# igd-geo/schwarzwald

Hardware: AMD Instinct MI355X
Metric: Mpoints/s end-to-end tile (Morton+sort+sample) (higher is better)
Workload: dtype u64 keys / f64 positions

## Files before the change

### schwarzwald_amd/csrc/swz_level.h

```cpp
#pragma once
#include "swz_device.h"
#include "swz_internal.h"

namespace swz {

enum : uint8_t { MODE_TAKE_ALL = 0, MODE_SAMPLE = 1 };

enum {
  CTR_NUM_NODES = 0,
  CTR_SAMPLE_NODES = 1,
  CTR_SAMPLE_POINTS = 2,
  CTR_ERROR = 3,
  CTR_REMAINING = 4,
  CTR_NUM_CELLS = 5,
  CTR_DONE_CELLS = 6,
  CTR_Q0 = 8,
  CTR_DBG_TIME = 20,
  CTR_DBG_TMAX = 21,
  CTR_DBG_HIST = 22,
  CTR_COUNT = 40
};

struct ActiveSet {
  const uint64_t* akey = nullptr;
// ... 59 lines not shown

LevelPlan make_plan(int level, int sampler, uint64_t max_points, float spacing_at_root, uint32_t max_depth,
                    const double bmin[3], const double bmax[3], bool force_sample, bool tiler_rules);
int alloc_level_buffers(swz_ctx* c, uint32_t m, LevelBuffers* lb);
int required_depth_host(int sampler, int node_level, double root_extent_x, float root_max_spacing);
int level_step(swz_ctx* c, const LevelPlan& plan, const ActiveSet& as, const SortedPoints& sp, const LevelBuffers& lb,
               int8_t* level_out, uint64_t* okey, uint32_t* oidx, LevelResult* res);
int fast_start_level(swz_ctx* c, const uint64_t* d_keys_sorted, uint32_t n, uint32_t concurrency, int* start_level);
int fast_prefix_counts(swz_ctx* c, const uint64_t* d_keys_sorted, uint32_t n, uint32_t* counts_host);
int fast_start_level_from_counts(const uint64_t* counts, uint32_t concurrency);

int min_distance_level(swz_ctx* c, const LevelPlan& plan, const ActiveSet& as, const SortedPoints& sp,
                       const LevelBuffers& lb, uint32_t num_nodes, uint32_t sample_nodes,
                       uint32_t sample_points, uint32_t* rounds_out);

int min_distance_property_level(swz_ctx* c, const LevelPlan& plan, const ActiveSet& as, const SortedPoints& sp,
                                const LevelBuffers& lb, uint32_t num_nodes, uint32_t sample_nodes,
                                uint32_t sample_points, uint32_t* phases_out);

struct MdPeerView {
  const uint4* rec = nullptr;
  const uint64_t* qpos = nullptr;
  const uint8_t* state = nullptr;
  const float4* ovf = nullptr;
  const uint32_t* gridmap = nullptr;
  const uint32_t* round_word = nullptr;
  const uint32_t* perm = nullptr;
  const double* xyz = nullptr;
  const uint32_t* aidx = nullptr;
  uint32_t ncells = 0, rg = 0, cell_shift = 0;
  uint32_t npoints = 0;
  int status = 0;
  int entered = 0;
};
struct MdShardRoot {
  int shard = 0, shards = 1;
  MdPeerView* views = nullptr;
  void (*barrier)(void*) = nullptr;
  void* barrier_arg = nullptr;
};

struct KeyMetric {
  bool ok = false;
  double T = 0.0;
  float f_lo = 0.f;
  float f_hi = 0.f;
};
KeyMetric key_metric(const swz_ctx* c, const LevelPlan& plan, const SortedPoints& sp);
int key_point_ids(swz_ctx* c, const ActiveSet& as, const SortedPoints& sp, const uint32_t** ids);
bool min_distance_level_uses_keys(const swz_ctx* c, const LevelPlan& plan, const SortedPoints& sp);
bool level_decides_on_keys(const swz_ctx* c, const LevelPlan& plan, const SortedPoints& sp);
int min_distance_keys_level(swz_ctx* c, const LevelPlan& plan, const ActiveSet& as, const SortedPoints& sp,
                            const LevelBuffers& lb, uint32_t num_nodes, uint32_t sample_nodes, uint32_t sample_points,
                            const uint32_t* snode_of, int cl, double typical_pop, uint32_t* rounds_out, bool* used,
                            const MdShardRoot* shard_root = nullptr);

int min_distance_rounds_level(swz_ctx* c, const LevelPlan& plan, const ActiveSet& as, const SortedPoints& sp, const LevelBuffers& lb,
                              uint32_t num_nodes, uint32_t sample_nodes, uint32_t sample_points, const uint32_t* snode_of, uint32_t* rounds_out,
                              bool* used);

int min_distance_sparse_level(swz_ctx* c, const LevelPlan& plan, const ActiveSet& as, const SortedPoints& sp,
                              const LevelBuffers& lb, const uint32_t* snode_of, bool all_sampled, uint32_t num_nodes,
                              uint32_t sample_nodes, uint32_t sample_points, const uint32_t occupied[12], uint32_t* rounds_out,
                              bool* used);

int min_distance_block_level(swz_ctx* c, const LevelPlan& plan, const ActiveSet& as, const SortedPoints& sp, const LevelBuffers& lb,
                             const uint32_t* snode_of, bool all_sampled, uint32_t num_nodes, uint32_t sample_nodes,
                             uint32_t sample_points, const uint32_t occupied[12], const KeyMetric& km, bool* done);

}
```

### schwarzwald_amd/csrc/swz_mdkeys.hip

```cpp
#include <algorithm>
#include <chrono>
#include <cmath>
#include <cstdio>
#include <cstdlib>
#include <cstring>
#include <string>
#include <vector>

#include "swz_level.h"
#include "swz_scan.h"

namespace swz {

constexpr uint32_t QNONE = 0xFFFFFFFFu;
constexpr unsigned long long QEMPTY = ~0ull;
constexpr uint32_t MQ_WOKEN = 0x80000000u;
constexpr int MQ_LIST_CAP = 128;
constexpr int MQ_FRESH_CAP = 32;
#ifndef MQ_MINW4
#define MQ_MINW4 4
#endif
#ifndef MQ_MINW1
#define MQ_MINW1 6
#endif
// ... 32 lines not shown
  return k;
}

__global__ __launch_bounds__(256) void mq_point_ids_kernel(const uint32_t* __restrict__ aidx, const uint32_t* __restrict__ perm, uint32_t m,
                                                           uint32_t ghosts, uint32_t* __restrict__ ids) {
  const uint32_t i = blockIdx.x * 256 + threadIdx.x;
  if (i >= m) return;
  const uint32_t s = aidx ? aidx[i] : i;
  ids[i] = s < ghosts ? perm[s] : ghosts + perm[s];
}
int key_point_ids(swz_ctx* c, const ActiveSet& as, const SortedPoints& sp, const uint32_t** ids) {
  if (!as.aidx && !sp.ghosts) {
    *ids = sp.perm;
    return SWZ_OK;
  }
  uint32_t* d = nullptr;
  SWZ_TRY(c->get("md_qids", (size_t)as.m, &d));
  hipLaunchKernelGGL(mq_point_ids_kernel, dim3(div_up(as.m, 256)), dim3(256), 0, c->stream, as.aidx, sp.perm, as.m, sp.ghosts, d);
  SWZ_LAUNCH_CHECK(c);
  *ids = d;
  return SWZ_OK;
}

constexpr uint32_t MQ_PEER_SHIFT = 28;
constexpr uint32_t MQ_ID_MASK = (1u << MQ_PEER_SHIFT) - 1u;
struct MqPeers {
  const uint4* rec[8];
  const uint64_t* qpos[8];
  const uint8_t* state[8];
  const float4* ovf[8];
  const uint32_t* gridmap[8];
  const uint32_t* round_word[8];
  const uint32_t* perm[8];
  const double* xyz[8];
  const uint32_t* aidx[8];
  uint32_t shard, shards;
};

struct MqArgs {
  const uint64_t* akey;
  const uint32_t* aidx;
  uint32_t m;
  const uint32_t* nid;
  const uint8_t* nmode;
  const uint32_t* nstart;
  const double* xyz;
  const uint32_t* perm;
  const double* gxyz;
  uint32_t ng;
  uint8_t* taken;
  uint32_t* counters;
  uint64_t* qpos;
  uint8_t* state;
  uint2* cinfo;
  uint32_t* crel;
  uint32_t* csnode;
  uint32_t* gridmap;
  uint32_t* qnbr;
  uint4* rec;
  float4* ovf;
  unsigned long long* slot;
  uint4* qst;
  uint32_t* queue[2];
  uint32_t* qctr;
  uint32_t* qtotal;
  uint32_t* qhead;
  uint32_t nseg, nseg_shift, segcap;
  const uint32_t* snode_of;
  uint32_t cell_shift;
  uint64_t cells_per_node;
  uint32_t cell_bits;
  uint32_t cell_levels;
  uint32_t rg, rg2_shift;
  float f_lo, f_hi;
  double sq_spacing;
  uint32_t patient;
  float lazy_frac;
  uint32_t all_sampled;
  uint32_t group, groups;
  uint32_t no_dead_test;
  uint32_t stats;
  uint32_t chain;
  uint32_t dense_min;
  uint8_t* dirty;
  uint32_t* bulk_round;
  const uint32_t* dlist;
  uint32_t* round_word;
  MqPeers peers;
};

__device__ __forceinline__ uint32_t uni(uint32_t v) { return (uint32_t)__builtin_amdgcn_readfirstlane((int)v); }
__device__ __forceinline__ uint32_t qb_u32(uint32_t v, int src) { return (uint32_t)__builtin_amdgcn_readlane((int)v, src); }
__device__ __forceinline__ float qb_f32(float v, int src) {
  return __int_as_float(__builtin_amdgcn_readlane(__float_as_int(v), src));
}
__device__ __forceinline__ unsigned long long qb_u64(unsigned long long v, int src) {
  const uint32_t lo = qb_u32((uint32_t)v, src), hi = qb_u32((uint32_t)(v >> 32), src);
  return ((unsigned long long)hi << 32) | lo;
}
template <typename Op>
__device__ __forceinline__ uint32_t mq_wave_scan(uint32_t v, Op op, uint32_t identity) {
  v = op(v, (uint32_t)__builtin_amdgcn_update_dpp((int)identity, (int)v, 0x111, 0xF, 0xF, false));
  v = op(v, (uint32_t)__builtin_amdgcn_update_dpp((int)identity, (int)v, 0x112, 0xF, 0xF, false));
  v = op(v, (uint32_t)__builtin_amdgcn_update_dpp((int)identity, (int)v, 0x114, 0xF, 0xF, false));
  v = op(v, (uint32_t)__builtin_amdgcn_update_dpp((int)identity, (int)v, 0x118, 0xF, 0xF, false));
  v = op(v, (uint32_t)__builtin_amdgcn_update_dpp((int)identity, (int)v, 0x142, 0xA, 0xF, false));
// ... 55 lines not shown
__device__ __forceinline__ uint32_t mq_ld_sys(const uint32_t* p) { return __hip_atomic_load(p, __ATOMIC_RELAXED, __HIP_MEMORY_SCOPE_SYSTEM); }

__device__ __forceinline__ bool mq_exact_near_peer(const MqArgs& a, uint32_t i, uint32_t j, uint32_t tag) {
  const double* p = sorted_point_xyz(a.xyz, a.perm, a.gxyz, a.ng, a.aidx ? a.aidx[i] : i);
  const double* q = tag ? a.peers.xyz[tag - 1u] + (size_t)a.peers.perm[tag - 1u][a.peers.aidx[tag - 1u] ? a.peers.aidx[tag - 1u][j] : j] * 3
                        : sorted_point_xyz(a.xyz, a.perm, a.gxyz, a.ng, a.aidx ? a.aidx[j] : j);
  return sq_dist(p[0], p[1], p[2], q[0], q[1], q[2]) < a.sq_spacing;
}

struct MqLds {
  uint4* stage;
  float4* list;
  float4* fresh;
  uint8_t* tag;
  uint32_t* trust;
  uint32_t* sid;
};
constexpr uint32_t MQ_CHAIN = 8;
__host__ __device__ constexpr uint32_t mq_staged(bool peers) { return peers ? 27u : 20u; }
static inline size_t mq_lds_bytes(uint32_t rg, bool peers) {
  return (size_t)(mq_staged(peers) * 2u * rg + MQ_LIST_CAP + MQ_FRESH_CAP) * 16u + MQ_LIST_CAP + MQ_CHAIN * 4u + 128u;
}

__device__ __forceinline__ bool mq_is_head(const MqArgs& a, uint32_t i) {
  if (!a.all_sampled && a.nmode[a.nid[i]] != MODE_SAMPLE) return false;
  return i == 0 || ((a.akey[i] >> a.cell_shift) != (a.akey[i - 1] >> a.cell_shift));
}

__global__ __launch_bounds__(256) void mq_pack_kernel(const uint64_t* __restrict__ akey, uint32_t m, uint64_t* __restrict__ qpos,
                                                      uint8_t* __restrict__ state) {
  const uint32_t i = blockIdx.x * 256 + threadIdx.x;
  if (i >= m) return;
  qpos[i] = mq_pack(akey[i]);
  state[i] = QS_OPEN;
}

struct MqHeadF {
  MqArgs a;
  __device__ uint32_t operator()(uint32_t i) const { return mq_is_head(a, i) ? 1u : 0u; }
};
struct MqCellBuildG {
  MqArgs a;
  __device__ void operator()(uint32_t i, uint32_t c, uint32_t head) const {
    const uint64_t key = a.akey[i];
    a.qpos[i] = mq_pack(key);
    a.state[i] = QS_OPEN;
    if (!head) return;
    a.cinfo[c].x = i;
    a.crel[c] = (uint32_t)((key >> a.cell_shift) & (a.cells_per_node - 1ull));
    a.csnode[c] = a.all_sampled ? a.nid[i] : a.snode_of[a.nid[i]];
  }
};

__global__ __launch_bounds__(256) void mq_cell_end_kernel(MqArgs a, uint32_t ncells) {
  const uint32_t c = blockIdx.x * 256 + threadIdx.x;
  if (c >= ncells) return;
  const uint32_t s = a.cinfo[c].x;
  const uint32_t node_end = a.nstart[a.nid[s] + 1];
  const uint32_t next = (c + 1 < ncells) ? a.cinfo[c + 1].x : a.m;
  const uint32_t e = next < node_end ? next : node_end;
  a.cinfo[c].y = e;
  a.gridmap[(uint64_t)a.csnode[c] * a.cells_per_node + a.crel[c]] = c;
  uint4* r = a.rec + ((size_t)c << a.rg2_shift);
  r[0] = make_uint4(s, 0u, 0u, e);
  r[a.rg] = make_uint4(s, 0u, 1u, e);
  a.qst[c] = make_uint4(QNONE, 0u, 0u, 0u);
}

__device__ __forceinline__ void mq_wave_push(bool want, uint32_t value, uint32_t* qout, uint32_t* cout) {
  const uint64_t m = __ballot(want);
  if (!m) return;
  const int leader = __ffsll((unsigned long long)m) - 1;
  uint32_t base = 0;
  if ((int)lane_id() == leader) base = atomicAdd(cout, (uint32_t)__popcll(m));
  base = __shfl(base, leader, WAVE);
  if (want) qout[base + (uint32_t)__popcll(m & lanemask_lt())] = value;
}

struct MqStart {
  uint32_t* queue[8];
  uint32_t* qctr[8];
  uint32_t groups;
  uint32_t lazy;
};

__global__ __launch_bounds__(256) void mq_nbr_build_kernel(MqArgs a, uint32_t ncells, MqStart st) {
  for (uint64_t cbase = (uint64_t)blockIdx.x * 8u; cbase < ncells; cbase += (uint64_t)gridDim.x * 8u) {
    const uint32_t c = (uint32_t)cbase + threadIdx.x / 32u;
    const uint32_t k = threadIdx.x & 31u;
    const bool in = c < ncells;
    uint32_t nb = QNONE;
    if (in && k == 13u) {
      nb = c;
    } else if (in && k < 27u) {
      const uint32_t rel = a.crel[c];
      const uint32_t all = (uint32_t)(a.cells_per_node - 1ull);
      const uint32_t mz = all & 0x09249249u, my = mz << 1, mx = mz << 2;
      const uint32_t v[3] = {rel & mx, rel & my, rel & mz};
      const uint32_t mk[3] = {mx, my, mz};
      const uint32_t d[3] = {k / 9u, (k / 3u) % 3u, k % 3u};
      bool inside = true;
      uint32_t nrel = 0;
#pragma unroll
      for (int ax = 0; ax < 3; ++ax) {
        uint32_t w = v[ax];
        if (d[ax] == 0u) {
          inside &= w != 0u;
          w = (w - 1u) & mk[ax];
        } else if (d[ax] == 2u) {
          inside &= w != mk[ax];
          w = ((w | ~mk[ax]) + 1u) & mk[ax];
        }
        nrel |= w;
      }
      if (inside) {
        if (a.peers.shards > 1u) {
          const uint32_t owner = (nrel >> (3u * (a.cell_levels - 1u))) * a.peers.shards / 8u;
          if (owner == a.peers.shard) {
            nb = a.gridmap[nrel];
          } else if (owner < a.peers.shard && a.peers.gridmap[owner]) {
            const uint32_t id = a.peers.gridmap[owner][nrel];
            if (id != QNONE) nb = ((owner + 1u) << MQ_PEER_SHIFT) | id;
          }
        } else {
          nb = a.gridmap[(uint64_t)a.csnode[c] * a.cells_per_node + nrel];
        }
      }
    }
    if (in) a.qnbr[(size_t)c * 32 + k] = nb;
    uint32_t best = 0;
    if (st.lazy && in && k < 27u && nb != QNONE && (a.peers.shards <= 1u || (nb >> MQ_PEER_SHIFT) == 0u) && nb < c) best = nb + 1u;
    if (st.lazy) {
#pragma unroll
      for (int off = 16; off >= 1; off >>= 1) best = max(best, (uint32_t)__shfl_xor((int)best, off, 32));
      if (in && best && nb + 1u == best) {
        const uint2 o = a.cinfo[best - 1u];
        const uint32_t bq = o.x + (uint32_t)((float)(o.y - 1u - o.x) * a.lazy_frac);
        a.slot[(size_t)(best - 1u) * 32 + (26u - k)] = (unsigned long long)bq;
        a.qst[c] = make_uint4(a.cinfo[c].x, k, bq, 0u);
      }
    }
    const bool push = in && k == 13u && best == 0u;
    const uint32_t seg = (uint32_t)(cbase >> 3) & (a.nseg - 1u);
    if (st.groups == 1u) {
      mq_wave_push(push, c | MQ_WOKEN, st.queue[0] + (size_t)seg * a.segcap, st.qctr[0] + (size_t)seg * 32u);
    } else {
      const uint32_t g = push ? a.csnode[c] % st.groups : 0u;
      for (uint32_t gg = 0; gg < st.groups; ++gg)
        mq_wave_push(push && g == gg, c | MQ_WOKEN, st.queue[gg] + (size_t)seg * a.segcap, st.qctr[gg] + (size_t)seg * 32u);
    }
  }
}

template <int SU>
__device__ __forceinline__ uint32_t mq_scan(const MqArgs& a, const uint64_t* __restrict__ qpos, const uint8_t* __restrict__ state,
                                            const MqLds& lds, uint32_t live_wn, uint32_t qs, uint32_t qe, float cx, float cy, float cz) {
  const uint32_t l = lane_id();
  for (uint32_t q0 = qs; q0 < qe; q0 += (uint32_t)SU * WAVE) {
    uint64_t v[SU];
    uint8_t s[SU];
#pragma unroll
    for (int u = 0; u < SU; ++u) {
      const uint32_t q = q0 + (uint32_t)u * WAVE + l;
      const bool inb = q < qe;
      v[u] = inb ? qpos[q] : 0ull;
      s[u] = inb ? state[q] : (uint8_t)QS_DEAD;
    }
#pragma unroll
    for (int u = 0; u < SU; ++u) {
      float x, y, z;
      mq_unpack(v[u], x, y, z);
      bool hit = s[u] != QS_DEAD && mq_d2(x, y, z, cx, cy, cz) < a.f_hi;
      uint64_t hb = __ballot(hit);
      if (hb && live_wn) {
        if (hit) {
          for (uint32_t i = 0; i < live_wn; ++i) {
            const float4 e = lds.list[i];
            if (mq_d2(x, y, z, e.x, e.y, e.z) < a.f_lo) {
              hit = false;
              break;
            }
          }
        }
        hb = __ballot(hit);
      }
      if (hb) return q0 + (uint32_t)u * WAVE + (uint32_t)__ffsll((unsigned long long)hb) - 1u;
    }
  }
  return QNONE;
}

__device__ __forceinline__ uint32_t mq_first_open(const uint8_t* __restrict__ state, uint32_t q0, uint32_t qe) {
  const uint32_t l = lane_id();
  while (q0 < qe) {
    const uint32_t base = q0 & ~15u;
    const uint32_t at = base + l * 16u;
    uint4 sb = make_uint4(0x02020202u, 0x02020202u, 0x02020202u, 0x02020202u);
    if (at < qe) sb = *reinterpret_cast<const uint4*>(state + at);
    const uint32_t w[4] = {sb.x, sb.y, sb.z, sb.w};
    uint32_t first = 16u;
// ... 644 lines not shown
    const uint32_t nb = a.qnbr[(size_t)c * 32 + tid];
    if (nb != QNONE && nb <= c) {
      const uint4* r = a.rec + ((size_t)nb << rg2s);
      const uint4 a0 = r[0], a1 = r[rg];
      const uint32_t pick = a1.z > a0.z ? 1u : 0u;
      const uint4 hd = pick ? a1 : a0;
      if (hd.z >= since && hd.y) {
        const uint32_t at = atomicAdd(&cnt, hd.y);
        for (uint32_t j = 0; j < hd.y && at + j < MQ_DENSE_LIST; ++j) {
          uint4 en;
          if (j < cap) en = r[pick * rg + 1u + j];
          else en = *reinterpret_cast<const uint4*>(a.ovf + (hd.w - 1u - (j - cap)));
          lst[at + j] = make_float4(__uint_as_float(en.x), __uint_as_float(en.y), __uint_as_float(en.z), 0.f);
        }
      }
    }
  }
  __syncthreads();
  const uint32_t n = cnt < MQ_DENSE_LIST ? cnt : MQ_DENSE_LIST;
  if (!n) return;
  for (uint32_t p = P + tid; p < e; p += 256u) {
    if (a.state[p] != QS_OPEN) continue;
    float x, y, z;
    mq_unpack(a.qpos[p], x, y, z);
    bool dead = false;
    for (uint32_t i = 0; i < n && !dead; ++i) dead = mq_d2(x, y, z, lst[i].x, lst[i].y, lst[i].z) < a.f_lo;
    if (dead) a.state[p] = QS_DEAD;
  }
}

__global__ void mq_round_word_kernel(uint32_t* word, uint32_t value) {
  __hip_atomic_store(word, value, __ATOMIC_RELAXED, __HIP_MEMORY_SCOPE_SYSTEM);
}

__global__ __launch_bounds__(256) void mq_verify_kernel(MqArgs a, uint32_t ncells, uint32_t* __restrict__ open_cells) {
  const uint32_t c = blockIdx.x * 256 + threadIdx.x;
  bool open = false;
  if (c < ncells) {
    const uint4* r = a.rec + ((size_t)c << a.rg2_shift);
    const uint4 h0 = r[0], h1 = r[a.rg];
    const uint4 h = h1.z > h0.z ? h1 : h0;
    open = h.x < h.w;
  }
  const uint64_t bm = __ballot(open);
  if (bm && lane_id() == 0) atomicAdd(open_cells, (uint32_t)__popcll(bm));
}

bool min_distance_level_uses_keys(const swz_ctx* c, const LevelPlan& plan, const SortedPoints& sp) {
  return key_metric(c, plan, sp).ok;
}

int min_distance_keys_level(swz_ctx* c, const LevelPlan& plan, const ActiveSet& as, const SortedPoints& sp, const LevelBuffers& lb,
                            uint32_t nnodes, uint32_t sample_nodes, uint32_t sample_points, const uint32_t* snode_of, int cl,
                            double typical_pop, uint32_t* rounds_out, bool* used, const MdShardRoot* shard_root) {
  *used = false;
  const KeyMetric km = key_metric(c, plan, sp);
  if (!km.ok) return SWZ_OK;
  const bool sharded = shard_root != nullptr && shard_root->shards > 1;
  const std::string sfx = sharded ? "_sr" : "";
  const uint32_t m = as.m;
  MqArgs a{};
  a.akey = as.akey;
  a.aidx = as.aidx;
  a.m = m;
  a.nid = lb.nid;
  a.nmode = lb.nmode;
  a.nstart = lb.nstart;
  a.xyz = sp.xyz;
  a.perm = sp.perm;
  a.gxyz = sp.ghost_xyz;
  a.ng = sp.ghosts;
  a.taken = lb.taken;
  a.counters = lb.counters;
  a.snode_of = snode_of;
  a.cells_per_node = 1ull << (3 * cl);
  a.cell_levels = (uint32_t)cl;
  a.peers.shards = sharded ? (uint32_t)shard_root->shards : 1u;
  a.peers.shard = sharded ? (uint32_t)shard_root->shard : 0u;
  a.cell_shift = (plan.node_shift == 63u ? 63u : plan.node_shift) - 3u * (uint32_t)cl;
  a.cell_bits = a.cell_shift / 3u;
  a.f_lo = km.f_lo;
  a.f_hi = km.f_hi;
  a.sq_spacing = plan.sq_spacing;
  a.all_sampled = sample_nodes == nnodes ? 1u : 0u;
  a.no_dead_test = c->opt_on("SWZ_MD_NO_DEAD_TEST", false) ? 1u : 0u;
  a.stats = c->opt("SWZ_MD_STATS") ? 1u : 0u;
  a.chain = std::min<uint32_t>(MQ_CHAIN, (uint32_t)std::max(1L, c->opt_int("SWZ_MD_CHAIN", 2)));
  if (a.cell_bits > 21u) return SWZ_OK;

  ProfScope ps(c, "sample_min_distance", (uint64_t)sample_points * 33ull, 1);
  uint32_t* d_cell_sums = nullptr;
  SWZ_TRY(fused_scan_sums(c, MqHeadF{a}, m, lb.counters + CTR_NUM_CELLS, "mqc", &d_cell_sums));
  uint32_t ncells = 0;
  SWZ_HIP(c, hipMemcpyAsync(&ncells, lb.counters + CTR_NUM_CELLS, 4, hipMemcpyDeviceToHost, c->stream));
  SWZ_HIP(c, hipStreamSynchronize(c->stream));
  *used = true;
  if (ncells == 0) return SWZ_OK;
  if (ncells >= 0x7FFFFFFFu) {
    *used = false;
    return SWZ_OK;
  }
  const double r_cell = std::ldexp(1.0, (int)a.cell_bits) / km.T;
  a.rg = (0.75 * r_cell * r_cell * r_cell <= 12.0) ? 4u : 8u;
  a.rg = c->opt_int("SWZ_MD_KEYS_RG", a.rg) >= 8 ? 8u : 4u;
  a.rg2_shift = a.rg == 4u ? 3u : 4u;

  SWZ_TRY(c->get(("md_qpos" + sfx).c_str(), (size_t)m, &a.qpos));
  SWZ_TRY(c->get(("md_qstate" + sfx).c_str(), (size_t)m, &a.state));
  SWZ_TRY(c->get(("md_qovf" + sfx).c_str(), (size_t)m, &a.ovf));
  SWZ_TRY(c->get(("md_qcinfo" + sfx).c_str(), (size_t)ncells, &a.cinfo));
  uint32_t* cellbuf = nullptr;
  SWZ_TRY(c->get(("md_qcells" + sfx).c_str(), (size_t)ncells * 2, &cellbuf));
  a.crel = cellbuf;
  a.csnode = cellbuf + ncells;
  SWZ_TRY(c->get(("md_qnbr" + sfx).c_str(), (size_t)ncells * 32, &a.qnbr));
  SWZ_TRY(c->get(("md_qrec" + sfx).c_str(), (size_t)ncells * 2 * a.rg, &a.rec));
  SWZ_TRY(c->get(("md_qslot" + sfx).c_str(), (size_t)ncells * 32, &a.slot));
  SWZ_TRY(c->get(("md_qst" + sfx).c_str(), (size_t)ncells, &a.qst));
  const uint64_t grid_entries = (uint64_t)sample_nodes * a.cells_per_node;
  SWZ_TRY(c->get(("md_gridmap" + sfx).c_str(), (size_t)grid_entries, &a.gridmap));
  SWZ_HIP(c, memset_large(a.gridmap, 0xFF, (size_t)grid_entries * 4, c->stream));
  SWZ_HIP(c, memset_large(a.slot, 0xFF, (size_t)ncells * 32 * sizeof(unsigned long long), c->stream));

  SWZ_TRY(fused_scan_apply(c, MqHeadF{a}, MqCellBuildG{a}, m, d_cell_sums));
  const uint32_t cb = div_up(ncells, 256);
  hipLaunchKernelGGL(mq_cell_end_kernel, dim3(cb), dim3(256), 0, c->stream, a, ncells);
  SWZ_LAUNCH_CHECK(c);
  struct WordGuard {
    swz_ctx* c;
    uint32_t* word = nullptr;
    bool done = false;
    ~WordGuard() {
      if (word && !done) {
        hipLaunchKernelGGL(mq_round_word_kernel, dim3(1), dim3(1), 0, c->stream, word, MQ_ROUND_FAILED);
        (void)hipStreamSynchronize(c->stream);
      }
    }
  } word_guard{c};
  if (sharded) {
    MdPeerView& mine = shard_root->views[shard_root->shard];
    int my_status = SWZ_OK;
    if (cl < 1 || ncells >= (1u << MQ_PEER_SHIFT) || sample_nodes != 1) my_status = SWZ_ERR_INTERNAL;
    const uint32_t* aidx_sr = nullptr;
    if (as.aidx) {
      uint32_t* cp = nullptr;
      SWZ_TRY(c->get("md_qaidx_sr", (size_t)m, &cp));
      SWZ_HIP(c, hipMemcpyAsync(cp, as.aidx, (size_t)m * 4, hipMemcpyDeviceToDevice, c->stream));
      aidx_sr = cp;
    }
    SWZ_TRY(c->get("md_qround_sr", (size_t)32, &a.round_word));
    hipLaunchKernelGGL(mq_round_word_kernel, dim3(1), dim3(1), 0, c->stream, a.round_word, MQ_FIRST_ROUND);
    SWZ_LAUNCH_CHECK(c);
    SWZ_HIP(c, hipStreamSynchronize(c->stream));
    mine.rec = a.rec;
    mine.qpos = a.qpos;
    mine.state = a.state;
    mine.ovf = a.ovf;
    mine.gridmap = a.gridmap;
    mine.round_word = a.round_word;
    mine.perm = a.perm;
    mine.xyz = a.xyz;
    mine.aidx = aidx_sr;
    mine.ncells = ncells;
    mine.npoints = m;
    mine.rg = a.rg;
    mine.cell_shift = a.cell_shift;
    mine.status = my_status;
    mine.entered = 1;
    word_guard.word = a.round_word;
    shard_root->barrier(shard_root->barrier_arg);
    for (int p = 0; p < shard_root->shards; ++p) {
      const MdPeerView& v = shard_root->views[p];
      if (v.status != SWZ_OK || (v.ncells && (v.rg != a.rg || v.cell_shift != a.cell_shift)))
        return c->fail(SWZ_ERR_INTERNAL, "MIN_DISTANCE root of a sharded batch: shard " + std::to_string(p) +
                                           " cannot take part in the joint sweep (cell levels, cell count or record size differ)");
      if (p < shard_root->shard && v.ncells) {
        a.peers.rec[p] = v.rec;
        a.peers.qpos[p] = v.qpos;
        a.peers.state[p] = v.state;
        a.peers.ovf[p] = v.ovf;
        a.peers.gridmap[p] = v.gridmap;
        a.peers.round_word[p] = v.round_word;
        a.peers.perm[p] = v.perm;
        a.peers.xyz[p] = v.xyz;
        a.peers.aidx[p] = v.aidx;
      }
    }
  }
  const bool many_small = ncells >= (4u << 20) && (double)sample_points / (double)ncells <= 128.0;
  a.patient = (uint32_t)c->opt_int("SWZ_MD_PATIENT", many_small ? 1 : 0);
  const bool lazy = c->opt_on("SWZ_MD_LAZY", true);
  a.lazy_frac = (float)c->opt_num("SWZ_MD_LAZY_FRAC", many_small ? 0.5 : 0.0);
  const bool big_cells = c->opt_on("SWZ_MD_BIG", typical_pop > 256.0);
  uint32_t groups = 1;
  if (sample_nodes >= 2 && !big_cells) groups = 2;
  groups = (uint32_t)std::max(1L, std::min(8L, c->opt_int("SWZ_MD_GROUPS", groups)));
  groups = std::min(groups, sample_nodes);
  if (sharded) groups = 1;
  uint32_t ndense = 0;
  a.dense_min = 0;
  a.dirty = nullptr;
  if (big_cells && groups == 1 && !sharded) {
    const uint32_t dense_min = (uint32_t)std::max(0L, c->opt_int("SWZ_MD_DENSE_MIN", 4096));
    if (dense_min && m >= dense_min) {
      uint32_t* dl = nullptr;
      uint32_t* dcount = nullptr;
      SWZ_TRY(c->get("md_qdense", (size_t)(m / dense_min + 1u), &dl));
      SWZ_TRY(c->get("md_qdense_count", (size_t)4, &dcount));
      SWZ_HIP(c, hipMemsetAsync(dcount, 0, 4, c->stream));
      a.dense_min = dense_min;
      hipLaunchKernelGGL(mq_dense_list_kernel, dim3(cb), dim3(256), 0, c->stream, a, ncells, dl, dcount);
      SWZ_LAUNCH_CHECK(c);
      SWZ_HIP(c, hipMemcpyAsync(&ndense, dcount, 4, hipMemcpyDeviceToHost, c->stream));
      SWZ_HIP(c, hipStreamSynchronize(c->stream));
      if (ndense) {
        SWZ_TRY(c->get("md_qdirty", (size_t)ncells, &a.dirty));
        SWZ_TRY(c->get("md_qbulk", (size_t)ncells, &a.bulk_round));
        SWZ_HIP(c, hipMemsetAsync(a.dirty, 0, (size_t)ncells, c->stream));
        SWZ_HIP(c, hipMemsetAsync(a.bulk_round, 0, (size_t)ncells * 4, c->stream));
        a.dlist = dl;
      } else {
        a.dense_min = 0;
      }
    }
  }
  a.nseg_shift = 5;
  a.nseg = 1u << a.nseg_shift;
  a.segcap = (uint32_t)std::min<uint64_t>(0x7FFFFFF0ull, 2ull * ncells / a.nseg + 4096ull);
  std::vector<MqArgs> ga(groups, a);
  std::vector<hipStream_t> gs(groups, c->stream);
  for (uint32_t g = 0; g < groups; ++g) {
    ga[g].group = g;
    ga[g].groups = groups;
    const std::string tag = std::to_string(g);
    SWZ_TRY(c->get(("md_qqueue0_g" + tag).c_str(), (size_t)a.nseg * a.segcap, &ga[g].queue[0]));
    SWZ_TRY(c->get(("md_qqueue1_g" + tag).c_str(), (size_t)a.nseg * a.segcap, &ga[g].queue[1]));
    SWZ_TRY(c->get(("md_qctr_g" + tag).c_str(), (size_t)6 * a.nseg * 32 + 32, &ga[g].qctr));
    ga[g].qhead = ga[g].qctr + (size_t)3 * a.nseg * 32;
    ga[g].qtotal = ga[g].qctr + (size_t)6 * a.nseg * 32;
    SWZ_HIP(c, hipMemsetAsync(ga[g].qctr, 0, ((size_t)6 * a.nseg * 32 + 32) * sizeof(uint32_t), c->stream));
    if (g > 0) {
      SWZ_TRY(c->get(("md_counters_g" + tag).c_str(), (size_t)CTR_COUNT, &ga[g].counters));
      SWZ_HIP(c, hipMemsetAsync(ga[g].counters, 0, CTR_COUNT * sizeof(uint32_t), c->stream));
      while (c->aux_streams.size() < g) {
        hipStream_t stn = nullptr;
        SWZ_HIP(c, hipStreamCreateWithFlags(&stn, hipStreamNonBlocking));
        c->aux_streams.push_back(stn);
      }
      gs[g] = c->aux_streams[g - 1];
    }
  }
  {
    MqStart start{};
    start.groups = groups;
    start.lazy = lazy ? 1u : 0u;
    for (uint32_t g = 0; g < groups; ++g) {
      start.queue[g] = ga[g].queue[0];
      start.qctr[g] = ga[g].qctr;
    }
    hipLaunchKernelGGL(mq_nbr_build_kernel, dim3(std::min<uint32_t>(div_up(ncells, 8), 1u << 20)), dim3(256), 0, c->stream, ga[0], ncells, start);
    SWZ_LAUNCH_CHECK(c);
    SWZ_STAGE(c, "mq tables");
  }
  const bool dbg = c->opt("SWZ_DEBUG") != nullptr;
  if (dbg)
    fprintf(stderr, "[swz] MIN_DISTANCE level %d on keys: %u pts in %u nodes, %u cells (cell levels %d), spacing %.1f key cells, band "
                    "[%.0f, %.0f), records of %u, typical cell %.0f pts, lazy %d (%.2f) patient %u groups %u big %d dense cells %u\n",
            plan.level, sample_points, sample_nodes, ncells, cl, km.T, (double)km.f_lo, (double)km.f_hi, a.rg - 1u, typical_pop, (int)lazy,
            (double)a.lazy_frac, a.patient, groups, (int)big_cells, ndense);
  hipEvent_t ev0 = nullptr, ev1 = nullptr;
  if (dbg) {
    ev0 = c->take_event();
    ev1 = c->take_event();
    (void)hipEventRecord(ev0, c->stream);
  }
  const size_t lds_bytes = mq_lds_bytes(a.rg, sharded);
  uint32_t sweep_grid = 0;
  {
    int dev = 0, cus = 0, per_cu = 0;
    (void)hipGetDevice(&dev);
    (void)hipDeviceGetAttribute(&cus, hipDeviceAttributeMultiprocessorCount, dev);
    const hipError_t oe = big_cells ? hipOccupancyMaxActiveBlocksPerMultiprocessor(&per_cu, mq_sweep_kernel<4, false>, WAVE, lds_bytes)
                                    : hipOccupancyMaxActiveBlocksPerMultiprocessor(&per_cu, mq_sweep_kernel<1, false>, WAVE, lds_bytes);
    if (oe != hipSuccess || per_cu < 1) per_cu = 8;
    if (cus < 1) cus = 256;
    uint32_t cap = (uint32_t)cus * (uint32_t)per_cu;
    if (const char* e = c->opt("SWZ_MD_GRID")) cap = (uint32_t)std::max(1, atoi(e)) * 4u;
    sweep_grid = std::max(a.nseg, (std::min<uint32_t>(cap / groups, ncells) + a.nseg - 1u) / a.nseg * a.nseg);
  }
  uint32_t batch = 32, batches_done = 0;
  const bool fixed_batch = c->opt("SWZ_MD_BATCH") != nullptr;
  if (fixed_batch) batch = std::max(1u, (uint32_t)c->opt_int("SWZ_MD_BATCH", 0));
  const auto wall0 = std::chrono::steady_clock::now();
  const double wall_limit = c->opt_num("SWZ_MD_TIME_LIMIT", 900.0);
  uint64_t max_rounds = 8ull * m + 1024;
  if (sharded) {
    uint64_t below = 0;
    for (int p = 0; p < shard_root->shard; ++p) below += shard_root->views[p].npoints;
    max_rounds += 64ull * below + 65536ull;
  }
  max_rounds = (uint64_t)c->opt_int("SWZ_MD_ROUND_LIMIT", (long)max_rounds);
  hipEvent_t fork = nullptr;
  if (groups > 1) {
    fork = c->take_event();
    SWZ_HIP(c, hipEventRecord(fork, c->stream));
    for (uint32_t g = 1; g < groups; ++g) SWZ_HIP(c, hipStreamWaitEvent(gs[g], fork, 0));
  }
  std::vector<uint32_t> gleft(groups, 1);
  uint32_t round = MQ_FIRST_ROUND;
  bool running = true;
  while (running) {
    for (uint32_t b = 0; b < batch; ++b, ++round) {
      for (uint32_t g = 0; g < groups; ++g) {
        if (sharded) {
          hipLaunchKernelGGL(mq_round_word_kernel, dim3(1), dim3(1), 0, gs[g], a.round_word, round);
          if (big_cells)
            hipLaunchKernelGGL((mq_sweep_kernel<4, true>), dim3(sweep_grid), dim3(WAVE), lds_bytes, gs[g], ga[g], round);
          else
            hipLaunchKernelGGL((mq_sweep_kernel<1, true>), dim3(sweep_grid), dim3(WAVE), lds_bytes, gs[g], ga[g], round);
        } else if (big_cells) {
          hipLaunchKernelGGL((mq_sweep_kernel<4, false>), dim3(sweep_grid), dim3(WAVE), lds_bytes, gs[g], ga[g], round);
// ... 87 lines not shown
```

### schwarzwald_amd/csrc/swz_mindist.hip

```cpp
#include <algorithm>
#include <chrono>
#include <cmath>
#include <cstdio>
#include <cstdlib>

#include "swz_level.h"
#include "swz_scan.h"

namespace swz {

constexpr uint32_t NONE32 = 0xFFFFFFFFu;
constexpr int MD_THREADS = 64;
constexpr int MD_WAVES = MD_THREADS / WAVE;
constexpr int MD_EXT_CAP = 128;
constexpr int MD_FRESH_CAP = 64;

enum : uint32_t { ST_STALLED = 0, ST_FINISHED = 1, ST_YIELD = 2 };

constexpr uint32_t MD_INLINE = 4;
struct alignas(128) MdCell {
  uint4 rec;
  uint4 cst;
  double acc[MD_INLINE][3];
};
// ... 757 lines not shown
    SWZ_HIP(c, hipStreamSynchronize(c->stream));
    for (int k = 0; k < 4; ++k) pop[k] = h[4] ? (double)h[k] / (double)h[4] : 1e30;
  }
  const double max_pop = 160.0;
  while (cl > 0 && plan.cell_levels_geo - cl < 3 && (double)sample_points / (double)std::max(1u, occupied[cl]) < per_cell &&
         pop[plan.cell_levels_geo - cl + 1] <= max_pop)
    --cl;
  while (cl > 0 && (double)sample_nodes * std::pow(8.0, cl) > 2147483648.0) --cl;
  if (const long coarsen = c->opt_int("SWZ_MD_COARSEN", 0))
    if (avg / std::pow(8.0, cl) >= c->opt_num("SWZ_MD_COARSEN_MIN", 32.0)) cl = std::max(0, cl - (int)coarsen);
  const uint64_t cells_per_node = 1ull << (3 * cl);

  MdArgs a{};
  a.akey = as.akey;
  a.aidx = as.aidx;
  a.m = m;
  a.nid = lb.nid;
  a.nmode = lb.nmode;
  a.nstart = lb.nstart;
  a.X = sp.X;
  a.Y = sp.Y;
  a.Z = sp.Z;
  a.taken = lb.taken;
  a.counters = lb.counters;
  a.cell_levels = (uint32_t)cl;
  a.cells_per_node = cells_per_node;
  a.cell_shift = (plan.node_shift == 63u ? 63u : plan.node_shift) - 3u * (uint32_t)cl;
  a.sq_spacing = plan.sq_spacing;
  a.all_sampled = sample_nodes == nnodes ? 1u : 0u;
  {
    const int cell_abs = plan.level + cl;
    const int sub = std::max(0, std::min(4, 20 - cell_abs));
    a.sub_levels = (uint32_t)sub;
    const double ext[3] = {plan.root.maxx - plan.root.minx, plan.root.maxy - plan.root.miny,
                           plan.root.maxz - plan.root.minz};
    for (int ax = 0; ax < 3; ++ax) {
      const double u = std::ldexp(ext[ax], -(plan.level + 1 + cl + sub));
      a.usq[ax] = u * u;
    }
    a.cull_sq = plan.sq_spacing * (1.0 + 0x1.0p-18);
    a.ff_min = (uint32_t)c->opt_int("SWZ_MD_FF_MIN", 1024);
    a.no_dead_test = c->opt_on("SWZ_MD_NO_DEAD_TEST", false) ? 1u : 0u;
    a.batch_blockers = (avg / std::pow(8.0, plan.cell_levels_geo) < 0.25) ? 1u : 0u;
  }

  uint32_t* snode = nullptr;
  SWZ_TRY(c->get("md_snode", (size_t)nnodes, &snode));
  a.snode_of = snode;
  hipLaunchKernelGGL(md_node_flag_kernel, dim3(div_up(nnodes, 256)), dim3(256), 0, c->stream, lb.nmode, nnodes, snode);
  SWZ_LAUNCH_CHECK(c);
  SWZ_TRY(scan_exclusive_u32(c, snode, snode, nnodes, nullptr, "mdn"));
  if (c->md_shard_root && plan.level == -1) {
    bool used = false;
    SWZ_TRY(min_distance_keys_level(c, plan, as, sp, lb, nnodes, sample_nodes, sample_points, snode, plan.cell_levels_geo, pop[0], rounds_out, &used,
                                    static_cast<const MdShardRoot*>(c->md_shard_root)));
    if (!used) return c->fail(SWZ_ERR_INTERNAL, "MIN_DISTANCE root of a sharded batch: the joint sweep needs a level that can be decided on keys");
    return SWZ_OK;
  }
  {
    bool used = false;
    SWZ_TRY(min_distance_sparse_level(c, plan, as, sp, lb, snode, sample_nodes == nnodes, nnodes, sample_nodes, sample_points, occupied, rounds_out, &used));
    if (used) return SWZ_OK;
  }
  {
    bool used = false;
    SWZ_TRY(min_distance_keys_level(c, plan, as, sp, lb, nnodes, sample_nodes, sample_points, snode, cl,
                                    pop[std::min(3, plan.cell_levels_geo - cl)], rounds_out, &used));
    if (used) return SWZ_OK;
  }
  if (!sp.X) return c->fail(SWZ_ERR_INTERNAL, "MIN_DISTANCE: this level needs the positions in Morton order and they were not gathered");
  if (as.aidx) {
    double *ax = nullptr, *ay = nullptr, *az = nullptr;
    SWZ_TRY(c->get("md_pos", (size_t)m * 3, &ax));
    ay = ax + m;
    az = ay + m;
    hipLaunchKernelGGL(md_gather_active_kernel, dim3(div_up(m, 256)), dim3(256), 0, c->stream, as.aidx, m, sp.X, sp.Y,
                       sp.Z, ax, ay, az);
    SWZ_LAUNCH_CHECK(c);
    a.X = ax;
    a.Y = ay;
    a.Z = az;
  }
  ProfScope ps(c, "sample_min_distance", (uint64_t)sample_points * 33ull, 1);

  uint32_t* d_cell_sums = nullptr;
  SWZ_TRY(fused_scan_sums(c, CellHeadF{a}, m, lb.counters + CTR_NUM_CELLS, "mdc", &d_cell_sums));
  uint32_t ncells = 0;
  SWZ_HIP(c, hipMemcpyAsync(&ncells, lb.counters + CTR_NUM_CELLS, 4, hipMemcpyDeviceToHost, c->stream));
  SWZ_HIP(c, hipStreamSynchronize(c->stream));
  if (ncells == 0) return SWZ_OK;

  uint32_t* cellbuf = nullptr;
  SWZ_TRY(c->get("md_cells", (size_t)ncells * 2, &cellbuf));
  uint32_t** fields[] = {&a.crel, &a.csnode};
  for (size_t f = 0; f < 2; ++f) *fields[f] = cellbuf + f * (size_t)ncells;
  SWZ_TRY(c->get("md_sleeper", (size_t)ncells * 28, &a.sleeper));
  SWZ_HIP(c, memset_large(a.sleeper, 0xFF, (size_t)ncells * 28 * sizeof(uint2), c->stream));
  SWZ_TRY(c->get("md_result", (size_t)ncells * 2, &a.result));
  SWZ_TRY(c->get("md_cell128", (size_t)ncells, &a.cells));
  SWZ_TRY(c->get("md_nbr_id", (size_t)ncells * 27, &a.nbr_id));
  SWZ_TRY(c->get("md_nbr_slot", (size_t)ncells * 32, &a.nbr_slot));
  SWZ_TRY(c->get("md_acc", (size_t)m * 3, &a.acc_xyz));
  SWZ_TRY(c->get("md_queue0", (size_t)ncells, &a.queue[0]));
  SWZ_TRY(c->get("md_queue1", (size_t)ncells, &a.queue[1]));
  const uint64_t grid_entries = (uint64_t)sample_nodes * cells_per_node;
  SWZ_TRY(c->get("md_gridmap", (size_t)grid_entries, &a.gridmap));
  SWZ_HIP(c, memset_large(a.gridmap, 0xFF, (size_t)grid_entries * 4, c->stream));

  SWZ_TRY(fused_scan_apply(c, CellHeadF{a}, CellBuildG{a}, m, d_cell_sums));
  const uint32_t cb = div_up(ncells, 256);
  hipLaunchKernelGGL(md_cell_end_kernel, dim3(cb), dim3(256), 0, c->stream, a, ncells);
  SWZ_LAUNCH_CHECK(c);
  SWZ_STAGE(c, "md cells");
  hipLaunchKernelGGL(md_nbr_build_kernel,
                     dim3(std::min<uint32_t>(div_up(ncells, 8), (uint32_t)c->opt_int("SWZ_MD_NBR_GRID", 1u << 20))),
                     dim3(256), 0, c->stream, a, ncells);
  SWZ_LAUNCH_CHECK(c);
  SWZ_STAGE(c, "md neighbour tables");
  const bool many_small = ncells >= (4u << 20) && (double)sample_points / (double)ncells <= 128.0;
  a.patient = (uint32_t)c->opt_int("SWZ_MD_PATIENT", many_small ? 1 : 0);
// ... 132 lines not shown
```

Baseline: 2393.

## Number min-distance cells directly by grid position when the grid is densely occupied

When estimated cell occupancy of the per-node grid is high, cells are indexed directly by (sample node, relative cell) instead of being compacted through a scan. This drops the fused scan pass, the device-to-host sync that read the cell count, the gridmap memset, and the gridmap and crel/csnode lookups. A new single kernel fills qpos, state and cell ranges, and neighbor lookups check the cinfo of the adjacent cell. The cost is that per-cell buffers and the sweep grid now cover empty cells too, so more memory is used and more cells are walked.

```diff
diff --git a/schwarzwald_amd/csrc/swz_level.h b/schwarzwald_amd/csrc/swz_level.h
--- a/schwarzwald_amd/csrc/swz_level.h
+++ b/schwarzwald_amd/csrc/swz_level.h
@@ -135,7 +135,8 @@
 bool level_decides_on_keys(const swz_ctx* c, const LevelPlan& plan, const SortedPoints& sp);
 int min_distance_keys_level(swz_ctx* c, const LevelPlan& plan, const ActiveSet& as, const SortedPoints& sp,
                             const LevelBuffers& lb, uint32_t num_nodes, uint32_t sample_nodes, uint32_t sample_points,
-                            const uint32_t* snode_of, int cl, double typical_pop, uint32_t* rounds_out, bool* used,
+                            const uint32_t* snode_of, int cl, double typical_pop, uint32_t est_cells, uint32_t* rounds_out,
+                            bool* used,
                             const MdShardRoot* shard_root = nullptr);
 
 int min_distance_rounds_level(swz_ctx* c, const LevelPlan& plan, const ActiveSet& as, const SortedPoints& sp, const LevelBuffers& lb,
diff --git a/schwarzwald_amd/csrc/swz_mdkeys.hip b/schwarzwald_amd/csrc/swz_mdkeys.hip
--- a/schwarzwald_amd/csrc/swz_mdkeys.hip
+++ b/schwarzwald_amd/csrc/swz_mdkeys.hip
@@ -108,6 +108,8 @@
   uint32_t* counters;
   uint64_t* qpos;
   uint8_t* state;
+  uint32_t direct;
+  uint32_t cpn_shift;
   uint2* cinfo;
   uint32_t* crel;
   uint32_t* csnode;
@@ -269,6 +271,51 @@
   }
 };
 
+__global__ __launch_bounds__(256) void mq_direct_build_kernel(MqArgs a, uint32_t vec) {
+  const uint64_t i0 = ((uint64_t)blockIdx.x * 256u + threadIdx.x) * 4u;
+  if (i0 >= a.m) return;
+  const uint32_t n = a.m - i0 < 4u ? (uint32_t)(a.m - i0) : 4u;
+  uint64_t key[6];
+  uint64_t q[4];
+  if (vec && n == 4u) {
+    const ulonglong2 v0 = *reinterpret_cast<const ulonglong2*>(a.akey + i0), v1 = *reinterpret_cast<const ulonglong2*>(a.akey + i0 + 2);
+    key[1] = v0.x, key[2] = v0.y, key[3] = v1.x, key[4] = v1.y;
+  } else {
+#pragma unroll
+    for (uint32_t j = 0; j < 4u; ++j) key[1 + j] = j < n ? a.akey[i0 + j] : 0ull;
+  }
+  key[0] = i0 ? a.akey[i0 - 1u] : 0ull;
+  key[5] = i0 + 4u < a.m ? a.akey[i0 + 4u] : 0ull;
+#pragma unroll
+  for (int j = 0; j < 4; ++j) q[j] = mq_pack(key[1 + j]);
+  if (n == 4u) {
+    ulonglong2 w0, w1;
+    w0.x = q[0], w0.y = q[1], w1.x = q[2], w1.y = q[3];
+    *reinterpret_cast<ulonglong2*>(a.qpos + i0) = w0;
+    *reinterpret_cast<ulonglong2*>(a.qpos + i0 + 2) = w1;
+    *reinterpret_cast<uint32_t*>(a.state + i0) = 0x01010101u * (uint32_t)QS_OPEN;
+  } else {
+    for (uint32_t j = 0; j < n; ++j) {
+      a.qpos[i0 + j] = q[j];
+      a.state[i0 + j] = QS_OPEN;
+    }
+  }
+#pragma unroll
+  for (uint32_t j = 0; j < 4u; ++j) {
+    if (j >= n) break;
+    const uint32_t i = (uint32_t)i0 + j;
+    const uint64_t pre = key[1 + j] >> a.cell_shift;
+    const bool first = i == 0u || (key[j] >> a.cell_shift) != pre;
+    const bool last = i + 1u == a.m || (key[2 + j] >> a.cell_shift) != pre;
+    if (!first && !last) continue;
+    const uint32_t node = a.nid[i];
+    if (!a.all_sampled && a.nmode[node] != MODE_SAMPLE) continue;
+    const uint64_t g = ((uint64_t)(a.all_sampled ? node : a.snode_of[node]) << a.cpn_shift) | (pre & (a.cells_per_node - 1ull));
+    if (first) a.cinfo[g].x = i;
+    if (last) a.cinfo[g].y = i + 1u;
+  }
+}
+
 __global__ __launch_bounds__(256) void mq_cell_end_kernel(MqArgs a, uint32_t ncells) {
   const uint32_t c = blockIdx.x * 256 + threadIdx.x;
   if (c >= ncells) return;
@@ -305,12 +352,18 @@
   for (uint64_t cbase = (uint64_t)blockIdx.x * 8u; cbase < ncells; cbase += (uint64_t)gridDim.x * 8u) {
     const uint32_t c = (uint32_t)cbase + threadIdx.x / 32u;
     const uint32_t k = threadIdx.x & 31u;
-    const bool in = c < ncells;
+    const bool in_grid = c < ncells;
+    bool in = in_grid;
+    if (a.direct && in_grid) {
+      const uint2 ci = a.cinfo[c];
+      if (k < 2u) a.rec[((size_t)c << a.rg2_shift) + k * a.rg] = make_uint4(ci.x, 0u, k, ci.y);
+      in = ci.x != ci.y;
+    }
     uint32_t nb = QNONE;
     if (in && k == 13u) {
       nb = c;
     } else if (in && k < 27u) {
-      const uint32_t rel = a.crel[c];
+      const uint32_t rel = a.direct ? (c & (uint32_t)(a.cells_per_node - 1ull)) : a.crel[c];
       const uint32_t all = (uint32_t)(a.cells_per_node - 1ull);
       const uint32_t mz = all & 0x09249249u, my = mz << 1, mx = mz << 2;
       const uint32_t v[3] = {rel & mx, rel & my, rel & mz};
@@ -339,6 +392,10 @@
             const uint32_t id = a.peers.gridmap[owner][nrel];
             if (id != QNONE) nb = ((owner + 1u) << MQ_PEER_SHIFT) | id;
           }
+        } else if (a.direct) {
+          const uint32_t g = (c - rel) | nrel;
+          const uint2 cn = a.cinfo[g];
+          if (cn.x != cn.y) nb = g;
         } else {
           nb = a.gridmap[(uint64_t)a.csnode[c] * a.cells_per_node + nrel];
         }
@@ -357,12 +414,13 @@
         a.qst[c] = make_uint4(a.cinfo[c].x, k, bq, 0u);
       }
     }
+    if (a.direct && in_grid && k == 2u && best == 0u) a.qst[c] = make_uint4(QNONE, 0u, 0u, 0u);
     const bool push = in && k == 13u && best == 0u;
     const uint32_t seg = (uint32_t)(cbase >> 3) & (a.nseg - 1u);
     if (st.groups == 1u) {
       mq_wave_push(push, c | MQ_WOKEN, st.queue[0] + (size_t)seg * a.segcap, st.qctr[0] + (size_t)seg * 32u);
     } else {
-      const uint32_t g = push ? a.csnode[c] % st.groups : 0u;
+      const uint32_t g = push ? (a.direct ? c >> a.cpn_shift : a.csnode[c]) % st.groups : 0u;
       for (uint32_t gg = 0; gg < st.groups; ++gg)
         mq_wave_push(push && g == gg, c | MQ_WOKEN, st.queue[gg] + (size_t)seg * a.segcap, st.qctr[gg] + (size_t)seg * 32u);
     }
@@ -1113,7 +1171,7 @@
 
 int min_distance_keys_level(swz_ctx* c, const LevelPlan& plan, const ActiveSet& as, const SortedPoints& sp, const LevelBuffers& lb,
                             uint32_t nnodes, uint32_t sample_nodes, uint32_t sample_points, const uint32_t* snode_of, int cl,
-                            double typical_pop, uint32_t* rounds_out, bool* used, const MdShardRoot* shard_root) {
+                            double typical_pop, uint32_t est_cells, uint32_t* rounds_out, bool* used, const MdShardRoot* shard_root) {
   *used = false;
   const KeyMetric km = key_metric(c, plan, sp);
   if (!km.ok) return SWZ_OK;
@@ -1135,6 +1193,7 @@
   a.counters = lb.counters;
   a.snode_of = snode_of;
   a.cells_per_node = 1ull << (3 * cl);
+  a.cpn_shift = 3u * (uint32_t)cl;
   a.cell_levels = (uint32_t)cl;
   a.peers.shards = sharded ? (uint32_t)shard_root->shards : 1u;
   a.peers.shard = sharded ? (uint32_t)shard_root->shard : 0u;
@@ -1150,43 +1209,74 @@
   if (a.cell_bits > 21u) return SWZ_OK;
 
   ProfScope ps(c, "sample_min_distance", (uint64_t)sample_points * 33ull, 1);
-  uint32_t* d_cell_sums = nullptr;
-  SWZ_TRY(fused_scan_sums(c, MqHeadF{a}, m, lb.counters + CTR_NUM_CELLS, "mqc", &d_cell_sums));
-  uint32_t ncells = 0;
-  SWZ_HIP(c, hipMemcpyAsync(&ncells, lb.counters + CTR_NUM_CELLS, 4, hipMemcpyDeviceToHost, c->stream));
-  SWZ_HIP(c, hipStreamSynchronize(c->stream));
-  *used = true;
-  if (ncells == 0) return SWZ_OK;
-  if (ncells >= 0x7FFFFFFFu) {
-    *used = false;
-    return SWZ_OK;
-  }
   const double r_cell = std::ldexp(1.0, (int)a.cell_bits) / km.T;
   a.rg = (0.75 * r_cell * r_cell * r_cell <= 12.0) ? 4u : 8u;
   a.rg = c->opt_int("SWZ_MD_KEYS_RG", a.rg) >= 8 ? 8u : 4u;
   a.rg2_shift = a.rg == 4u ? 3u : 4u;
+  const uint64_t grid_entries = (uint64_t)sample_nodes * a.cells_per_node;
+  {
+    const size_t per_cell = sizeof(uint2) + 32u * 4u + 2u * a.rg * sizeof(uint4) + 32u * 8u + sizeof(uint4) + 5u;
+    uint64_t max_cells = 0x7FFFFFF0ull;
+    if (const char* mc = c->opt("SWZ_MD_DIRECT_MAX_CELLS")) {
+      max_cells = std::min<uint64_t>(max_cells, (uint64_t)std::max(0LL, atoll(mc)));
+    } else {
+      size_t free_b = 0, total_b = 0, held = 0;
+      if (hipMemGetInfo(&free_b, &total_b) != hipSuccess) free_b = 0;
+      for (const auto& kv : c->bufs)
+        if (!kv.second.host && kv.first.compare(0, 4, "md_q") == 0) held += kv.second.cap;
+      max_cells = std::min<uint64_t>(max_cells, (uint64_t)((double)(free_b + held) * 0.9 / (double)per_cell));
+    }
+    const double occupancy = (double)est_cells / (double)std::max<uint64_t>(1, grid_entries);
+    bool direct = occupancy >= c->opt_num("SWZ_MD_DIRECT_MIN_OCCUPANCY", 0.5);
+    if (const char* f = c->opt("SWZ_MD_DIRECT")) direct = atoi(f) != 0;
+    a.direct = (direct && !sharded && grid_entries <= max_cells) ? 1u : 0u;
+  }
+  *used = true;
+  uint32_t ncells = 0;
+  uint32_t* d_cell_sums = nullptr;
+  if (a.direct) {
+    if (sample_points == 0) return SWZ_OK;
+    ncells = (uint32_t)grid_entries;
+  } else {
+    SWZ_TRY(fused_scan_sums(c, MqHeadF{a}, m, lb.counters + CTR_NUM_CELLS, "mqc", &d_cell_sums));
+    SWZ_HIP(c, hipMemcpyAsync(&ncells, lb.counters + CTR_NUM_CELLS, 4, hipMemcpyDeviceToHost, c->stream));
+    SWZ_HIP(c, hipStreamSynchronize(c->stream));
+    if (ncells == 0) return SWZ_OK;
+    if (ncells >= 0x7FFFFFFFu) {
+      *used = false;
+      return SWZ_OK;
+    }
+  }
+  const uint32_t occ_cells = a.direct ? std::max(1u, std::min<uint32_t>(est_cells, ncells)) : ncells;
 
   SWZ_TRY(c->get(("md_qpos" + sfx).c_str(), (size_t)m, &a.qpos));
   SWZ_TRY(c->get(("md_qstate" + sfx).c_str(), (size_t)m, &a.state));
   SWZ_TRY(c->get(("md_qovf" + sfx).c_str(), (size_t)m, &a.ovf));
   SWZ_TRY(c->get(("md_qcinfo" + sfx).c_str(), (size_t)ncells, &a.cinfo));
-  uint32_t* cellbuf = nullptr;
-  SWZ_TRY(c->get(("md_qcells" + sfx).c_str(), (size_t)ncells * 2, &cellbuf));
-  a.crel = cellbuf;
-  a.csnode = cellbuf + ncells;
+  if (!a.direct) {
+    uint32_t* cellbuf = nullptr;
+    SWZ_TRY(c->get(("md_qcells" + sfx).c_str(), (size_t)ncells * 2, &cellbuf));
+    a.crel = cellbuf;
+    a.csnode = cellbuf + ncells;
+  }
   SWZ_TRY(c->get(("md_qnbr" + sfx).c_str(), (size_t)ncells * 32, &a.qnbr));
   SWZ_TRY(c->get(("md_qrec" + sfx).c_str(), (size_t)ncells * 2 * a.rg, &a.rec));
   SWZ_TRY(c->get(("md_qslot" + sfx).c_str(), (size_t)ncells * 32, &a.slot));
   SWZ_TRY(c->get(("md_qst" + sfx).c_str(), (size_t)ncells, &a.qst));
-  const uint64_t grid_entries = (uint64_t)sample_nodes * a.cells_per_node;
-  SWZ_TRY(c->get(("md_gridmap" + sfx).c_str(), (size_t)grid_entries, &a.gridmap));
-  SWZ_HIP(c, memset_large(a.gridmap, 0xFF, (size_t)grid_entries * 4, c->stream));
   SWZ_HIP(c, memset_large(a.slot, 0xFF, (size_t)ncells * 32 * sizeof(unsigned long long), c->stream));
-
-  SWZ_TRY(fused_scan_apply(c, MqHeadF{a}, MqCellBuildG{a}, m, d_cell_sums));
   const uint32_t cb = div_up(ncells, 256);
-  hipLaunchKernelGGL(mq_cell_end_kernel, dim3(cb), dim3(256), 0, c->stream, a, ncells);
-  SWZ_LAUNCH_CHECK(c);
+  if (a.direct) {
+    SWZ_HIP(c, memset_large(a.cinfo, 0, (size_t)ncells * sizeof(uint2), c->stream));
+    hipLaunchKernelGGL(mq_direct_build_kernel, dim3(div_up(m, 1024)), dim3(256), 0, c->stream, a,
+                       ((uintptr_t)a.akey & 15u) == 0 ? 1u : 0u);
+    SWZ_LAUNCH_CHECK(c);
+  } else {
+    SWZ_TRY(c->get(("md_gridmap" + sfx).c_str(), (size_t)grid_entries, &a.gridmap));
+    SWZ_HIP(c, memset_large(a.gridmap, 0xFF, (size_t)grid_entries * 4, c->stream));
+    SWZ_TRY(fused_scan_apply(c, MqHeadF{a}, MqCellBuildG{a}, m, d_cell_sums));
+    hipLaunchKernelGGL(mq_cell_end_kernel, dim3(cb), dim3(256), 0, c->stream, a, ncells);
+    SWZ_LAUNCH_CHECK(c);
+  }
   struct WordGuard {
     swz_ctx* c;
     uint32_t* word = nullptr;
@@ -1248,7 +1338,7 @@
       }
     }
   }
-  const bool many_small = ncells >= (4u << 20) && (double)sample_points / (double)ncells <= 128.0;
+  const bool many_small = occ_cells >= (4u << 20) && (double)sample_points / (double)occ_cells <= 128.0;
   a.patient = (uint32_t)c->opt_int("SWZ_MD_PATIENT", many_small ? 1 : 0);
   const bool lazy = c->opt_on("SWZ_MD_LAZY", true);
   a.lazy_frac = (float)c->opt_num("SWZ_MD_LAZY_FRAC", many_small ? 0.5 : 0.0);
@@ -1325,9 +1415,9 @@
   }
   const bool dbg = c->opt("SWZ_DEBUG") != nullptr;
   if (dbg)
-    fprintf(stderr, "[swz] MIN_DISTANCE level %d on keys: %u pts in %u nodes, %u cells (cell levels %d), spacing %.1f key cells, band "
+    fprintf(stderr, "[swz] MIN_DISTANCE level %d on keys: %u pts in %u nodes, %u cells%s (cell levels %d), spacing %.1f key cells, band "
                     "[%.0f, %.0f), records of %u, typical cell %.0f pts, lazy %d (%.2f) patient %u groups %u big %d dense cells %u\n",
-            plan.level, sample_points, sample_nodes, ncells, cl, km.T, (double)km.f_lo, (double)km.f_hi, a.rg - 1u, typical_pop, (int)lazy,
+            plan.level, sample_points, sample_nodes, ncells, a.direct ? " of the grid, numbered directly" : "", cl, km.T, (double)km.f_lo, (double)km.f_hi, a.rg - 1u, typical_pop, (int)lazy,
             (double)a.lazy_frac, a.patient, groups, (int)big_cells, ndense);
   hipEvent_t ev0 = nullptr, ev1 = nullptr;
   if (dbg) {
diff --git a/schwarzwald_amd/csrc/swz_mindist.hip b/schwarzwald_amd/csrc/swz_mindist.hip
--- a/schwarzwald_amd/csrc/swz_mindist.hip
+++ b/schwarzwald_amd/csrc/swz_mindist.hip
@@ -833,7 +833,7 @@
   SWZ_TRY(scan_exclusive_u32(c, snode, snode, nnodes, nullptr, "mdn"));
   if (c->md_shard_root && plan.level == -1) {
     bool used = false;
-    SWZ_TRY(min_distance_keys_level(c, plan, as, sp, lb, nnodes, sample_nodes, sample_points, snode, plan.cell_levels_geo, pop[0], rounds_out, &used,
+    SWZ_TRY(min_distance_keys_level(c, plan, as, sp, lb, nnodes, sample_nodes, sample_points, snode, plan.cell_levels_geo, pop[0], occupied[plan.cell_levels_geo], rounds_out, &used,
                                     static_cast<const MdShardRoot*>(c->md_shard_root)));
     if (!used) return c->fail(SWZ_ERR_INTERNAL, "MIN_DISTANCE root of a sharded batch: the joint sweep needs a level that can be decided on keys");
     return SWZ_OK;
@@ -846,7 +846,7 @@
   {
     bool used = false;
     SWZ_TRY(min_distance_keys_level(c, plan, as, sp, lb, nnodes, sample_nodes, sample_points, snode, cl,
-                                    pop[std::min(3, plan.cell_levels_geo - cl)], rounds_out, &used));
+                                    pop[std::min(3, plan.cell_levels_geo - cl)], occupied[cl], rounds_out, &used));
     if (used) return SWZ_OK;
   }
   if (!sp.X) return c->fail(SWZ_ERR_INTERNAL, "MIN_DISTANCE: this level needs the positions in Morton order and they were not gathered");
```

New measurement: 2480, median of 6. +3.6%, better.
